# kakaobrain/rq-vae-transformer

Hardware: NVIDIA H100
Metric: 256x256 images/sec (ImageNet 1.4B RQ-Transformer, 8x8x4 codes, K=16384, top-k 1024, sample+decode) (higher is better)
Workload: dtype fp16

## Files before the change

include/rqb200.h:

```cpp
#ifndef RQB200_H
#define RQB200_H

#include <stddef.h>
#include <stdint.h>

#ifdef __cplusplus
extern "C" {
#endif

#define RQB200_OK 0
#define RQB200_EINVAL (-1)
#define RQB200_ECUDA (-2)
#define RQB200_ENODEV (-3)
#define RQB200_EWORKSPACE (-4)
#define RQB200_ESTATE (-5)

#define RQB200_F32 0
#define RQB200_BF16 1
#define RQB200_F16 2
#define RQB200_E4M3 3

#define RQB200_MODE_EXACT 0
#define RQB200_MODE_FAST 1

// ... 121 lines not shown
int64_t rqb200_vae_last_launches(const rqb200_vae* h);

int rqb200_dbg_gemm_tc(const void* W16, const void* X16, const float* bias, const float* residual, void* out,
                       int out_is_16, int gelu, float* partial, int N_out, int K, int B, int splits, int fmt, void* stream);
int rqb200_dbg_gemm_tc_fp8(const void* W8_packed, const float* scale, const void* X16, const float* bias, const float* residual,
                           void* out, int out_is_16, int gelu, float* partial, int N_out, int K, int B, int splits, void* stream);

int rqb200_dbg_rq_quantize(int form, const float* x, const float* codebook, int64_t N, int K, int C, int D, int64_t* codes,
                           float* quant_list, float* residual_out, void* stream);
int rqb200_dbg_rq_quantize_depthwise(int form, const float* x, const float* const* codebooks_host, const int32_t* K_host, int64_t N,
                                     int C, int D, int64_t* codes, float* quant_list, float* residual_out, void* stream);
int rqb200_dbg_sample_logits(int algo, const float* logits, const float* q, int B, int V, float temperature, int top_k,
                             float top_p, int64_t* out_idx, void* stream);

int rqb200_dbg_conv_tc(const void* X16, const void* W16, const void* X16lo, const void* W16lo, const float* bias,
                       const float* residual, float* out, int B, int H, int W, int Cin, int Cout, int ks, int out_nchw,
                       void* stream);

int rqb200_dbg_conv_tc_gn(const void* X16, const void* W16, const void* X16lo, const void* W16lo, const float* bias,
                          const float* residual, float* out, double* gn_part, int B, int H, int W, int Cin, int Cout, int ks,
                          int out_nchw, void* stream);

int rqb200_dbg_rows_gemm(const void* X16, const void* W16, const float* bias, const float* residual, float* out_f32, void* out_16,
                         int gelu, int fmt, int64_t M, int N_out, int K, void* stream);

int rqb200_dbg_log_prob_rows(const float* logits, int64_t ld, int V, int64_t rows, const int64_t* targets, float* out, void* stream);

int rqb200_dbg_attn_step(int form, const float* part, int S, const float* bqkv, void* kc, void* vc, void* att, int B, int E, int Tmax,
                         const int* t_dev, int t_host, int fmt, void* stream);
int rqb200_dbg_prefill_attn(const void* qkv, void* kc, void* vc, void* att, int G, int T, int E, int Tmax, int fmt, void* stream);
int rqb200_dbg_ln(int form, const float* x_in, const float* part, int S, const float* bias, const float* extra, float* x_out, const float* g,
                  const float* b, void* xn, int64_t rows, int E, int fmt, void* stream);
int rqb200_dbg_act_reduce(const float* part, int S, const float* bias, void* h, int B, int N, int fmt, void* stream);

int rqb200_dbg_vae_conv(const float* X, const void* Wt, int wdtype, const float* bias, const float* residual, float* out, int B, int H,
                        int W, int Cin, int Cout, int ks, int stride, int upsample, int in_nchw, int out_nchw, void* stream);
int rqb200_dbg_groupnorm(int form, const float* X, const float* gamma, const float* beta, float* Y, void* Y16, void* Y16lo,
                         double* stats_ws, int64_t ws_doubles, int B, int HW, int C, int silu, void* stream);
int rqb200_dbg_cast_f16(const float* X, void* Y16, void* Y16lo, int B, int H, int W, int C, int upsample, void* stream);
int rqb200_dbg_vae_attn(const float* qkv, float* out, int B, int HW, int C, void* stream);

#ifdef __cplusplus
}
#endif
#endif
```

rq-vae-transformer_b200/csrc/ar_fast.cu:

```cuda
#include <algorithm>
#include <cstring>
#include <string>
#include <vector>

#include "kernels.h"
#include "tc_common.cuh"

namespace rqb {

#define TR_IN(tr)  do { if ((tr) != nullptr && blockIdx.x == 0 && threadIdx.x == 0) (tr)[0] = tc::gtimer(); } while (0)
#define TR_DEP(tr) do { if ((tr) != nullptr && blockIdx.x == 0 && threadIdx.x == 0) (tr)[1] = tc::gtimer(); } while (0)
#define TR_OUT(tr) do { if ((tr) != nullptr && blockIdx.x == 0 && threadIdx.x == 0) { (tr)[2] = tc::gtimer(); (tr)[3] = (tr)[2]; } } while (0)

struct PrefetchList {
    const void* p[8];
    uint32_t bytes[8];
    int n;
};

template <int THREADS, int NCH>
__global__ void __launch_bounds__(THREADS)
ln_reduce_kernel(const float* __restrict__ x_in, const float* __restrict__ partial, int S, const float* __restrict__ bias,
                 const float* __restrict__ extra, float* __restrict__ x_out, const float* __restrict__ g,
                 const float* __restrict__ be, h16* __restrict__ xn, int B, int E, int bf, long long* tr, PrefetchList pf) {
    __shared__ float red[33];
    tc::pdl_launch_dependents();
    TR_IN(tr);
    if (blockIdx.x == 0 && threadIdx.x < pf.n) tc::bulk_prefetch_l2(pf.p[threadIdx.x], pf.bytes[threadIdx.x]);
    tc::pdl_wait();
    TR_DEP(tr);
    const int b = blockIdx.x;
    const int E4 = E >> 2;
    const int S12 = S < 12 ? S : 12;
    float4 v[NCH], gg[NCH], bb[NCH];
    float s = 0.f;
#pragma unroll
    for (int k = 0; k < NCH; k++) {
        const int e4 = threadIdx.x + k * THREADS;
        v[k] = make_float4(0.f, 0.f, 0.f, 0.f);
        if (e4 < E4) {
            float4 pr[12];
            if (xn) { gg[k] = reinterpret_cast<const float4*>(g)[e4]; bb[k] = reinterpret_cast<const float4*>(be)[e4]; }
#pragma unroll
            for (int i = 0; i < 12; i++)
                if (i < S12) pr[i] = reinterpret_cast<const float4*>(partial + ((int64_t)i * B + b) * E)[e4];
            if (x_in) v[k] = reinterpret_cast<const float4*>(x_in + (int64_t)b * E)[e4];
            if (bias) { float4 t = reinterpret_cast<const float4*>(bias)[e4]; v[k].x += t.x; v[k].y += t.y; v[k].z += t.z; v[k].w += t.w; }
#pragma unroll
            for (int i = 0; i < 12; i++)
                if (i < S12) { v[k].x += pr[i].x; v[k].y += pr[i].y; v[k].z += pr[i].z; v[k].w += pr[i].w; }
            for (int i = 12; i < S; i++) {
                float4 p0 = reinterpret_cast<const float4*>(partial + ((int64_t)i * B + b) * E)[e4];
                v[k].x += p0.x; v[k].y += p0.y; v[k].z += p0.z; v[k].w += p0.w;
            }
            if (extra) { float4 t = reinterpret_cast<const float4*>(extra)[e4]; v[k].x += t.x; v[k].y += t.y; v[k].z += t.z; v[k].w += t.w; }
            if (x_out) reinterpret_cast<float4*>(x_out + (int64_t)b * E)[e4] = v[k];
            s += (v[k].x + v[k].y) + (v[k].z + v[k].w);
        }
    }
    if (xn) {
        const float mean = block_sum(s, red) / (float)E;
        if (tr != nullptr && blockIdx.x == 0 && threadIdx.x == 0) tr[2] = tc::gtimer();
        float q = 0.f;
#pragma unroll
        for (int k = 0; k < NCH; k++)
            if (threadIdx.x + k * THREADS < E4) {
                const float d0 = v[k].x - mean, d1 = v[k].y - mean, d2 = v[k].z - mean, d3 = v[k].w - mean;
                q = fmaf(d0, d0, q); q = fmaf(d1, d1, q); q = fmaf(d2, d2, q); q = fmaf(d3, d3, q);
            }
        const float rstd = rsqrtf(block_sum(q, red) / (float)E + 1e-5f);
#pragma unroll
        for (int k = 0; k < NCH; k++) {
            const int e4 = threadIdx.x + k * THREADS;
            if (e4 < E4) {
                uint2 pk;
                pk.x = pack_h16x2((v[k].x - mean) * rstd * gg[k].x + bb[k].x, (v[k].y - mean) * rstd * gg[k].y + bb[k].y, bf);
                pk.y = pack_h16x2((v[k].z - mean) * rstd * gg[k].z + bb[k].z, (v[k].w - mean) * rstd * gg[k].w + bb[k].w, bf);
                reinterpret_cast<uint2*>(xn + (int64_t)b * E)[e4] = pk;
            }
        }
        if (tr != nullptr && blockIdx.x == 0 && threadIdx.x == 0) tr[3] = tc::gtimer();
    } else {
        TR_OUT(tr);
    }
}

template <int NV>
__global__ void __launch_bounds__(256)
ln_rows_kernel(const float* __restrict__ x_in, const float* __restrict__ extra, float* __restrict__ x_out, const float* __restrict__ g,
               const float* __restrict__ be, h16* __restrict__ xn, int64_t M, int E, int bf) {
    tc::pdl_launch_dependents();
    tc::pdl_wait();
    const int lane = threadIdx.x & 31;
// ... 157 lines not shown
    m = warp_max(m);
    if (tr != nullptr && blockIdx.x == 0 && threadIdx.x == 0) tr[2] = tc::gtimer();
    float sum = 0.f;
    for (int j = lane; j < t; j += 32) {
        float e = __expf(ps[j] - m);
        ps[j] = e;
        sum += e;
    }
    const float e_new = __expf(s_new - m);
    sum = warp_sum(sum) + e_new;
    __syncwarp();
    const float inv = 1.0f / sum;
    float2 o = make_float2(e_new * vf.x, e_new * vf.y);
    for (int j0 = 0; j0 < t; j0 += 64) {
        if (j0 > 0) {
#pragma unroll
            for (int u = 0; u < 64; u++)
                raw[u] = (j0 + u < t) ? *reinterpret_cast<const uint32_t*>(vb + (int64_t)(j0 + u) * 64 + 2 * lane) : 0u;
        }
#pragma unroll
        for (int u = 0; u < 64; u++)
            if (j0 + u < t) {
                const float2 vv = unpack_h16x2(raw[u], bf);
                o.x = fmaf(ps[j0 + u], vv.x, o.x);
                o.y = fmaf(ps[j0 + u], vv.y, o.y);
            }
    }
    *reinterpret_cast<uint32_t*>(att + (int64_t)b * E + c) = pack_h16x2(o.x * inv, o.y * inv, bf);
    }
    if (tr != nullptr && blockIdx.x == 0 && threadIdx.x == 0) tr[3] = tc::gtimer();
}

constexpr int AF2_MAXROWS = 320;
static size_t attn2_smem(int rows) { return (size_t)rows * 256 + ((size_t)rows + 64 * 3 + 4 * 64 + 8) * sizeof(float); }
__device__ __forceinline__ void cp_async16(uint32_t dst, const void* src) {
    asm volatile("cp.async.cg.shared.global [%0], [%1], 16;" ::"r"(dst), "l"(src) : "memory");
}
__global__ void __launch_bounds__(128, 11)
attn_fast2_kernel(const float* __restrict__ part, int S, const float* __restrict__ bqkv, h16* __restrict__ kc, h16* __restrict__ vc,
                  h16* __restrict__ att, int B, int E, int nh, int Tmax, int rows, const int* __restrict__ t_ptr, int t_host, int bf,
                  long long* tr) {
    extern __shared__ __align__(128) uint8_t af2_smem[];
    uint8_t* Ks = af2_smem;
    uint8_t* Vs = Ks + (size_t)rows * 128;
    float* ps = reinterpret_cast<float*>(Vs + (size_t)rows * 128);
    float* qs = ps + rows;
    float* kn = qs + 64;
    float* vn = kn + 64;
    float* ov = vn + 64;
    float* red = ov + 256;
    const int lane = threadIdx.x & 31, w = threadIdx.x >> 5;
    tc::pdl_launch_dependents();
    TR_IN(tr);
    tc::pdl_wait();
    TR_DEP(tr);
    const int b = blockIdx.x / nh, h = blockIdx.x % nh;
    const int t = t_ptr ? *t_ptr : t_host;
    h16* kb = kc + ((int64_t)(b * nh + h) * Tmax) * 64;
    h16* vb = vc + ((int64_t)(b * nh + h) * Tmax) * 64;
    {
        const uint32_t ks = tc::smem_u32(Ks), vs = tc::smem_u32(Vs);
        for (int i = threadIdx.x; i < t * 8; i += 128) {
            const int j = i >> 3, c = i & 7;
            const uint32_t off = (uint32_t)j * 128u + (uint32_t)((c ^ (j & 7)) << 4);
            cp_async16(ks + off, kb + (int64_t)j * 64 + c * 8);
            cp_async16(vs + off, vb + (int64_t)j * 64 + c * 8);
        }
        asm volatile("cp.async.commit_group;" ::: "memory");
    }
    if (w < 3) {
        const int c = h * 64 + 2 * lane;
        float2 a = make_float2(bqkv[w * E + c], bqkv[w * E + c + 1]);
#pragma unroll 4
        for (int s = 0; s < S; s++) {
            const float2 pp = *reinterpret_cast<const float2*>(part + ((int64_t)s * B + b) * 3 * E + w * E + c);
            a.x += pp.x; a.y += pp.y;
        }
        const uint32_t a2 = pack_h16x2(a.x, a.y, bf);
        const float2 af = unpack_h16x2(a2, bf);
        float* dst = w == 0 ? qs : (w == 1 ? kn : vn);
        dst[2 * lane] = af.x;
        dst[2 * lane + 1] = af.y;
        if (w == 1) *reinterpret_cast<uint32_t*>(kb + (int64_t)t * 64 + 2 * lane) = a2;
        if (w == 2) *reinterpret_cast<uint32_t*>(vb + (int64_t)t * 64 + 2 * lane) = a2;
    }
    asm volatile("cp.async.wait_group 0;" ::: "memory");
    __syncthreads();
    const float s_new = warp_sum(qs[2 * lane] * kn[2 * lane] + qs[2 * lane + 1] * kn[2 * lane + 1]) * 0.125f;
    float m = -INFINITY;
    {
        const int half = threadIdx.x & 1;
        for (int j0 = 0; j0 < t; j0 += 64) {
            const int j = j0 + (threadIdx.x >> 1);
            float acc = 0.f;
            if (j < t) {
#pragma unroll
                for (int i = 0; i < 4; i++) {
                    const int c = half * 4 + i;
                    const uint4 k4 = *reinterpret_cast<const uint4*>(Ks + (size_t)j * 128 + ((c ^ (j & 7)) << 4));
                    const float4 qa = *reinterpret_cast<const float4*>(qs + c * 8), qb = *reinterpret_cast<const float4*>(qs + c * 8 + 4);
                    float2 kk = unpack_h16x2(k4.x, bf);
                    acc = fmaf(qa.x, kk.x, acc); acc = fmaf(qa.y, kk.y, acc);
                    kk = unpack_h16x2(k4.y, bf);
                    acc = fmaf(qa.z, kk.x, acc); acc = fmaf(qa.w, kk.y, acc);
                    kk = unpack_h16x2(k4.z, bf);
                    acc = fmaf(qb.x, kk.x, acc); acc = fmaf(qb.y, kk.y, acc);
                    kk = unpack_h16x2(k4.w, bf);
                    acc = fmaf(qb.z, kk.x, acc); acc = fmaf(qb.w, kk.y, acc);
                }
            }
            acc += __shfl_xor_sync(0xffffffffu, acc, 1);
            acc *= 0.125f;
            if (j < t) {
                if (half == 0) ps[j] = acc;
                m = fmaxf(m, acc);
            }
        }
    }
    m = warp_max(m);
    if (lane == 0) red[w] = m;
    __syncthreads();
    m = fmaxf(fmaxf(fmaxf(red[0], red[1]), fmaxf(red[2], red[3])), s_new);
    if (tr != nullptr && blockIdx.x == 0 && threadIdx.x == 0) tr[2] = tc::gtimer();
    float sum = 0.f;
    for (int j = threadIdx.x; j < t; j += 128) {
        const float e = __expf(ps[j] - m);
        ps[j] = e;
        sum += e;
    }
    sum = warp_sum(sum);
    if (lane == 0) red[4 + w] = sum;
    __syncthreads();
    const float e_new = __expf(s_new - m);
    const float inv = 1.0f / ((((red[4] + red[5]) + red[6]) + red[7]) + e_new);
    float2 o = w == 0 ? make_float2(e_new * vn[2 * lane], e_new * vn[2 * lane + 1]) : make_float2(0.f, 0.f);
    for (int j = w; j < t; j += 4) {
        const uint32_t v2 = *reinterpret_cast<const uint32_t*>(Vs + (size_t)j * 128 + (((lane >> 2) ^ (j & 7)) << 4) + ((lane & 3) << 2));
        const float2 vv = unpack_h16x2(v2, bf);
        const float pj = ps[j];
        o.x = fmaf(pj, vv.x, o.x);
        o.y = fmaf(pj, vv.y, o.y);
    }
    ov[w * 64 + 2 * lane] = o.x;
    ov[w * 64 + 2 * lane + 1] = o.y;
    __syncthreads();
    if (w == 0) {
        const float ox = ((ov[2 * lane] + ov[64 + 2 * lane]) + ov[128 + 2 * lane]) + ov[192 + 2 * lane];
        const float oy = ((ov[2 * lane + 1] + ov[64 + 2 * lane + 1]) + ov[128 + 2 * lane + 1]) + ov[192 + 2 * lane + 1];
        *reinterpret_cast<uint32_t*>(att + (int64_t)b * E + h * 64 + 2 * lane) = pack_h16x2(ox * inv, oy * inv, bf);
    }
    if (tr != nullptr && blockIdx.x == 0 && threadIdx.x == 0) tr[3] = tc::gtimer();
}

template <bool BF>
__device__ __forceinline__ void pa_mma(float (&c)[4], const uint32_t (&a)[4], uint32_t b0, uint32_t b1) {
    if (BF)
        asm volatile("mma.sync.aligned.m16n8k16.row.col.f32.bf16.bf16.f32 {%0,%1,%2,%3}, {%4,%5,%6,%7}, {%8,%9}, {%0,%1,%2,%3};"
                     : "+f"(c[0]), "+f"(c[1]), "+f"(c[2]), "+f"(c[3]) : "r"(a[0]), "r"(a[1]), "r"(a[2]), "r"(a[3]), "r"(b0), "r"(b1));
    else
        asm volatile("mma.sync.aligned.m16n8k16.row.col.f32.f16.f16.f32 {%0,%1,%2,%3}, {%4,%5,%6,%7}, {%8,%9}, {%0,%1,%2,%3};"
                     : "+f"(c[0]), "+f"(c[1]), "+f"(c[2]), "+f"(c[3]) : "r"(a[0]), "r"(a[1]), "r"(a[2]), "r"(a[3]), "r"(b0), "r"(b1));
}
__device__ __forceinline__ void pa_ldsm4(uint32_t (&r)[4], uint32_t addr) {
    asm volatile("ldmatrix.sync.aligned.m8n8.x4.shared.b16 {%0,%1,%2,%3}, [%4];" : "=r"(r[0]), "=r"(r[1]), "=r"(r[2]), "=r"(r[3]) : "r"(addr));
}
__device__ __forceinline__ void pa_ldsm4_t(uint32_t (&r)[4], uint32_t addr) {
    asm volatile("ldmatrix.sync.aligned.m8n8.x4.trans.shared.b16 {%0,%1,%2,%3}, [%4];" : "=r"(r[0]), "=r"(r[1]), "=r"(r[2]), "=r"(r[3]) : "r"(addr));
}
// ... 354 lines not shown
    w.kc_body = a.take<h16>(per_body * c.n_body);
    w.vc_body = a.take<h16>(per_body * c.n_body);
    w.kc_head = a.take<h16>(per_head * c.n_head_layers);
    w.vc_head = a.take<h16>(per_head * c.n_head_layers);
    w.Mmax = f.batched_prefill ? (int64_t)B * prefill_tmax(c) : 0;
    const int64_t Mp = w.Mmax ? w.Mmax + 128 : 0;
    w.PX = a.take<float>(Mp * E);
    w.PXN = a.take<h16>(Mp * E);
    w.PQKV = a.take<h16>(Mp * 3 * E);
    w.PATT = a.take<h16>(Mp * E);
    w.PH = a.take<h16>(Mp * 4 * E);
    w.PS = a.take<h16>(w.Mmax * c.code_dim);
    if (ws) *ws = w;
    return a.off + 256;
}

static int gemm_w(const ArFast& f, const StreamedWeight& w, const CUtensorMap& tx, GemmTcParams p, bool pdl, cudaStream_t st) {
    p.fmt = f.bf; p.ld_out = w.N_out;
    return launch_gemm_tc(w, tx, p, pdl, st);
}

static int gemm(const ArFast& f, const char* name, const StreamedWeight& w, const CUtensorMap& tx, int B, int splits, int mode, const float* bias,
                float bias_scale, void* out, float* partial, const float* residual, int64_t ld_res, const int* res_row_ptr,
                int64_t res_row_stride, cudaStream_t st) {
    GemmTcParams p = {};
    p.B = B; p.splits = splits; p.mode = mode;
    p.bias = bias; p.bias_scale = bias_scale; p.out = out; p.partial = partial;
    p.residual = residual; p.ld_res = ld_res; p.res_row_ptr = res_row_ptr; p.res_row_stride = res_row_stride;
    p.trace = tr_slot(f, name);
    return gemm_w(f, w, tx, p, f.use_pdl, st);
}


static int ln(int rows, const float* x_in, const float* partial, int S, const float* bias, const float* extra, float* x_out, const float* g,
              const float* be, h16* xn, int E, int bf, bool pdl, long long* tr, const PrefetchList& pf, cudaStream_t st) {
    return launch_pdl(ln_reduce_kernel<384, 3>, dim3((unsigned)rows), dim3(384), (size_t)0, st, pdl, x_in, partial, S, bias, extra, x_out,
                      g, be, xn, rows, E, bf, tr, pf);
}

static int attn_form(int Tmax) { return Tmax >= 16 && Tmax - 1 <= AF2_MAXROWS ? 2 : 1; }

static int attn(int form, const float* part, int S, const float* bqkv, h16* kc, h16* vc, h16* att, int B, int E, int Tmax, const int* t_ptr,
                int t_host, int bf, bool pdl, long long* tr, cudaStream_t st) {
    const int nh = E / 64;
    if (form == 0) form = attn_form(Tmax);
    if (form == 2) {
        const int rows = (Tmax - 1 + 7) & ~7;
        RQB_ENSURE_SMEM(attn2_smem(AF2_MAXROWS), attn_fast2_kernel);
        {
            static std::atomic<uint64_t> carve{0};
            int dev = 0;
            RQB_CUDA(cudaGetDevice(&dev));
            if (!(carve.load(std::memory_order_acquire) & (1ull << (dev & 63)))) {
                RQB_CUDA(cudaFuncSetAttribute(attn_fast2_kernel, cudaFuncAttributePreferredSharedMemoryCarveout, 100));
                carve.fetch_or(1ull << (dev & 63), std::memory_order_release);
            }
        }
        return launch_pdl(attn_fast2_kernel, dim3((unsigned)(B * nh)), dim3(128), attn2_smem(rows), st, pdl, part, S, bqkv, kc, vc, att, B, E,
                          nh, Tmax, rows, t_ptr, t_host, bf, tr);
    }
    const size_t smem = (size_t)(4 * ((Tmax + 31) & ~31)) * sizeof(float);
    return launch_pdl(attn_fast_kernel, dim3((unsigned)ceil_div(B * nh, 4)), dim3(128), smem, st, pdl, part, S, bqkv, kc, vc, att, B, E, nh,
                      Tmax, t_ptr, t_host, bf, tr);
}

static int act_reduce(const float* partial, int S, const float* bias, h16* h, int B, int N, int bf, bool pdl, long long* tr, cudaStream_t st) {
    return launch_pdl(act_reduce_kernel, dim3((unsigned)std::min<int64_t>(ceil_div((int64_t)B * N / 4, 256), 1184)), dim3(256), (size_t)0, st,
                      pdl, partial, S, bias, h, B, N, bf, tr);
}

static int fast_stack(const ArFast& f, const std::vector<rqb200_block_weights>& blocks, const std::vector<FastLayer>& maps,
                      FastWs& ws, float* x, const float* pending_extra, const float* x_src, h16* kc, h16* vc, int Tmax,
                      const int* t_ptr, int t_host, const float* fin_g, const float* fin_b, cudaStream_t st) {
    const rqb200_ar_config& c = f.cfg;
    const int E = c.embed_dim, B = f.B;
    const int64_t per = (int64_t)B * c.n_head * Tmax * 64;
    const float* nof = nullptr;
    for (size_t l = 0; l < blocks.size(); l++) {
        const rqb200_block_weights& bw = blocks[l];
        const bool first = l == 0;
        const bool pend = l > 0;
        PrefetchList pf = {};
        if (l + 1 < blocks.size()) {
            const rqb200_block_weights& nx = blocks[l + 1];
            const void* ptrs[8] = {nx.ln1_w, nx.ln1_b, nx.bqkv, nx.bproj, nx.ln2_w, nx.ln2_b, nx.b1, bw.b2};
            const uint32_t words[8] = {(uint32_t)E, (uint32_t)E, (uint32_t)(3 * E), (uint32_t)E, (uint32_t)E, (uint32_t)E, (uint32_t)(4 * E),
                                       (uint32_t)E};
            for (int i = 0; i < 8; i++) { pf.p[i] = ptrs[i]; pf.bytes[i] = words[i] * 4u; }
            pf.n = 8;
        }
        RQB_TRY(ln(B, first ? x_src : x, pend ? ws.P : nof, pend ? f.split_fc2 : 0, pend ? blocks[l - 1].b2 : nof, first ? pending_extra : nof,
                   x, bw.ln1_w, bw.ln1_b, ws.XN, E, f.bf, f.use_pdl, tr_slot(f, "ln1"), pf, st));
        RQB_TRY(gemm(f, "qkv", maps[l].qkv, f.tx_xn, B, f.split_qkv, GT_PARTIAL, nullptr, 1.f, nullptr, ws.P, nullptr, 0, nullptr, 0, st));
        RQB_TRY(attn(0, ws.P, f.split_qkv, bw.bqkv, kc + per * l, vc + per * l, ws.ATT, B, E, Tmax, t_ptr, t_host, f.bf, f.use_pdl,
                     tr_slot(f, "attn"), st));
// ... 586 lines not shown
        return fail(RQB200_EINVAL, "dbg_prefill_attn: need fmt 0..1, G >= 1, 1 <= T <= 2048, E % 64 == 0");
    if (!qkv || !att || !kc != !vc) return fail(RQB200_EINVAL, "dbg_prefill_attn: null qkv / att, or only one of kc / vc");
    if (kc && T > Tmax) return fail(RQB200_EINVAL, "dbg_prefill_attn: T > Tmax");
    if (rqb200_device_count() <= 0) return fail(RQB200_ENODEV, "dbg_prefill_attn: no CUDA device");
    return prefill_attn((const h16*)qkv, (h16*)kc, (h16*)vc, (h16*)att, G, T, E, Tmax, fmt, false, (cudaStream_t)stream);
}

extern "C" int rqb200_dbg_ln(int form, const float* x_in, const float* partial, int S, const float* bias, const float* extra, float* x_out,
                             const float* g, const float* b, void* xn, int64_t rows, int E, int fmt, void* stream) {
    using namespace rqb;
    if (form < 0 || form > 2 || fmt < 0 || fmt > 1 || rows < 1 || rows > INT32_MAX || S < 0 || E < 128 || E % 128 || E > 4608)
        return fail(RQB200_EINVAL, "dbg_ln: need form 0..2, fmt 0..1, 1 <= rows < 2^31, S >= 0, E % 128 == 0, E <= 4608");
    if ((S > 0 && !partial) || (xn && (!g || !b))) return fail(RQB200_EINVAL, "dbg_ln: null partial, or xn without g / b");
    if (form != 1 && (S > 0 || partial || bias || !x_in))
        return fail(RQB200_EINVAL, "dbg_ln: forms 0 and 2 (the batched passes' LayerNorm) take x_in and no partials or bias");
    int dev = 0, n_sm = 0;
    if (rqb200_device_count() <= 0 || cudaGetDevice(&dev) != cudaSuccess ||
        cudaDeviceGetAttribute(&n_sm, cudaDevAttrMultiProcessorCount, dev) != cudaSuccess)
        return fail(RQB200_ENODEV, "dbg_ln: no CUDA device");
    const cudaStream_t st = (cudaStream_t)stream;
    if (form == 1) return ln((int)rows, x_in, partial, S, bias, extra, x_out, g, b, (h16*)xn, E, fmt, false, nullptr, PrefetchList{}, st);
    if (form == 2) return ln_rows_warp(rows, x_in, extra, x_out, g, b, (h16*)xn, E, fmt, n_sm, st);
    return ln_rows(rows, x_in, extra, x_out, g, b, (h16*)xn, E, fmt, n_sm, st);
}

extern "C" int rqb200_dbg_act_reduce(const float* partial, int S, const float* bias, void* h, int B, int N, int fmt, void* stream) {
    using namespace rqb;
    if (fmt < 0 || fmt > 1 || S < 0 || B < 1 || N < 4 || N % 4)
        return fail(RQB200_EINVAL, "dbg_act_reduce: need fmt 0..1, S >= 0, B >= 1, N % 4 == 0");
    if (!bias || !h || (S > 0 && !partial)) return fail(RQB200_EINVAL, "dbg_act_reduce: null argument");
    if (rqb200_device_count() <= 0) return fail(RQB200_ENODEV, "dbg_act_reduce: no CUDA device");
    return act_reduce(partial, S, bias, (h16*)h, B, N, fmt, false, nullptr, (cudaStream_t)stream);
}
```

rq-vae-transformer_b200/csrc/gemm_tc.cu:

```cuda
#include "kernels.h"
#include "tc_common.cuh"
#include <cudaTypedefs.h>
#include <cstdlib>

namespace rqb {

static int get_encode_fn(PFN_cuTensorMapEncodeTiled_v12000* fn) {
    static PFN_cuTensorMapEncodeTiled_v12000 cached = nullptr;
    if (!cached) {
        void* p = nullptr;
        cudaDriverEntryPointQueryResult q;
        cudaError_t e = cudaGetDriverEntryPoint("cuTensorMapEncodeTiled", &p, cudaEnableDefault, &q);
        if (e != cudaSuccess || q != cudaDriverEntryPointSuccess || !p)
            return fail(RQB200_ECUDA, "cuTensorMapEncodeTiled entry point not available");
        cached = (PFN_cuTensorMapEncodeTiled_v12000)p;
    }
    *fn = cached;
    return 0;
}

int make_tmap_2d(CUtensorMap* out, const void* base, int elem_bytes_log2, uint64_t inner, uint64_t outer,
                 uint64_t row_stride_bytes, uint32_t box_inner, uint32_t box_outer) {
    PFN_cuTensorMapEncodeTiled_v12000 enc;
    RQB_TRY(get_encode_fn(&enc));
// ... 254 lines not shown
        typename F::Frag none;
        for (int i = 0; i < nkb; i++) {
            const int s = i % STAGES;
            tc::mbar_wait(&full[s], (i / STAGES) & 1);
            tc::mbar_wait(&xfull[s], (i / STAGES) & 1);
            F::template kblock<BN>(acc, none, smem + s * STAGE_BYTES, wg, t, p.fmt, i == 0);
            tc::wgmma_commit();
            tc::wgmma_wait<1>();
            if (i > 0 && lane == 0) tc::mbar_arrive(&empty[(i - 1) % STAGES]);
        }
    }
    tc::wgmma_wait<0>();
    tc::acc_fence(acc);
    if (nkb > 0 && lane == 0) tc::mbar_arrive(&empty[(nkb - 1) % STAGES]);
    F::scale(acc, rs);

    tc::pdl_wait();
    if (tr && t == 0) p.trace[2] = tc::gtimer();
    const int nb = (p.B - m0) < BN ? (p.B - m0) : BN;
    const int n_base = tile * 128;
    tc::drain_acc<BN, CW, 0>(acc, stage, wg, t, [&p, n_base, split, m0, nb](const float (&v)[16], int r, int col0) {
        const int n = n_base + r;
        switch (p.mode) {
            case GT_PARTIAL: gt_epilogue<GT_PARTIAL>(p, v, n, split, m0, nb, col0); break;
            case GT_F32: gt_epilogue<GT_F32>(p, v, n, split, m0, nb, col0); break;
            case GT_H16: gt_epilogue<GT_H16>(p, v, n, split, m0, nb, col0); break;
            default: gt_epilogue<GT_H16_GELU>(p, v, n, split, m0, nb, col0); break;
        }
    });
    if (tr && t == 0) p.trace[3] = tc::gtimer();
}

template <int BN, int WF>
static int launch_gemm_tc_t(const typename GtFormat<WF>::Arg& w, const CUtensorMap& tmX, const GemmTcParams& p, bool pdl,
                            cudaStream_t st) {
    using F = GtFormat<WF>;
    constexpr size_t smem = (size_t)F::stages(BN) * (F::A_BYTES + BN * 128) + 128 * ((BN < 32 ? BN : 32) + 4) * 4 + 1024 + 512;
    static_assert(smem <= 227 * 1024, "gemm_tc: shared memory budget");
    RQB_ENSURE_SMEM(smem, gemm_tc_kernel<BN, WF>);
    return launch_pdl(gemm_tc_kernel<BN, WF>, dim3((unsigned)(ceil_div(p.N_out, 128) * p.splits), (unsigned)ceil_div(p.B, BN)),
                      dim3(GT_THREADS), smem, st, pdl, w, tmX, p);
}

template <int WF>
static int launch_gemm_tc_bn(const typename GtFormat<WF>::Arg& w, const CUtensorMap& tmX, const GemmTcParams& p, int bn, bool pdl,
                             cudaStream_t st) {
    switch (bn) {
        case 16: return launch_gemm_tc_t<16, WF>(w, tmX, p, pdl, st);
        case 32: return launch_gemm_tc_t<32, WF>(w, tmX, p, pdl, st);
        case 64: return launch_gemm_tc_t<64, WF>(w, tmX, p, pdl, st);
        case 128: return launch_gemm_tc_t<128, WF>(w, tmX, p, pdl, st);
        default: return launch_gemm_tc_t<(WF == GT_E4M3 ? 128 : 256), WF>(w, tmX, p, pdl, st);
    }
}

int make_streamed_weight(StreamedWeight* out, bool e4m3, const void* w, const float* scale, int N_out, int K) {
    *out = StreamedWeight{};
    out->N_out = N_out;
    out->K = K;
    if (e4m3) {
        if (w == nullptr || scale == nullptr || (reinterpret_cast<uintptr_t>(w) & 15) != 0)
            return fail(RQB200_EINVAL, "gemm_tc: packed E4M3 weights must be 16-byte aligned, scales non-null");
        out->q8 = static_cast<const uint8_t*>(w);
        out->s8 = scale;
        return 0;
    }
    out->w16 = w;
    return make_tmap_2d(&out->tm, w, 1, (uint64_t)K, (uint64_t)N_out, (uint64_t)K * 2, 64, 128);
}

int launch_gemm_tc(const StreamedWeight& w, const CUtensorMap& tmX, GemmTcParams p, bool pdl, cudaStream_t st) {
    p.N_out = w.N_out;
    p.K = w.K;
    if (p.K % 64 != 0 || p.N_out % 128 != 0) return fail(RQB200_EINVAL, "gemm_tc: need K % 64 == 0 and N_out % 128 == 0");
    if (p.B < 1) return fail(RQB200_EINVAL, "gemm_tc: no activation rows");
    if (p.splits < 1 || p.splits > p.K / 64) return fail(RQB200_EINVAL, "gemm_tc: bad split count");
    if (w.e4m3() && p.fmt != 0) return fail(RQB200_EINVAL, "gemm_tc: E4M3 weights take fp16 activations only");
    if (p.fmt != 0 && p.fmt != 1) return fail(RQB200_EINVAL, "gemm_tc: fmt must be 0 (fp16) or 1 (bf16)");
    if (p.B > 256 && p.mode == GT_PARTIAL) return fail(RQB200_EINVAL, "gemm_tc: split-K takes at most 256 activation rows");
    if (p.mode != GT_PARTIAL && p.splits != 1) return fail(RQB200_EINVAL, "gemm_tc: direct epilogues need splits == 1");
    const int bn = gemm_tc_chunk_rows(w, p.B);
    if (ceil_div(p.B, bn) > 65535) return fail(RQB200_EINVAL, "gemm_tc: more than 65535 row chunks");
    if (w.e4m3()) return launch_gemm_tc_bn<GT_E4M3>(GtE4m3Tiles{w.q8, w.s8}, tmX, p, bn, pdl, st);
    return launch_gemm_tc_bn<GT_W16>(w.tm, tmX, p, bn, pdl, st);
}
// ... 33 lines not shown
```

rq-vae-transformer_b200/csrc/kernels.h:

```cpp
#pragma once
#include <cuda.h>

#include "common.cuh"

namespace rqb {
constexpr int RQ_MAX_TABLES = 16;
struct RqTables {
    const float* cb[RQ_MAX_TABLES];
    int K[RQ_MAX_TABLES];
    int n;
    __host__ __device__ __forceinline__ int of(int depth) const { return n == 1 ? 0 : depth; }
};
int make_rq_tables(RqTables* out, const float* const* cb_host, const int32_t* K_host, int n);

int launch_rq_quantize(const float* x, const RqTables& tabs, int64_t N, int C, int D, int64_t* codes, float* quant_list,
                       float* resid_out, cudaStream_t st, int form = 0);
bool rq_quantize2_supported(int64_t N, const RqTables& tabs, int C);
int launch_rq_quantize2(const float* x, const RqTables& tabs, int64_t N, int C, int D, int64_t* codes, float* quant_list,
                        float* resid_out, cudaStream_t st);
int launch_rq_embed(const int64_t* codes, const RqTables& tabs, int64_t N, int D, int C, float* out, bool sum, cudaStream_t st);
int launch_sample(const float* logits, const float* q, int B, int V, float temperature, int top_k, float top_p,
                  int64_t* out_idx, const int64_t* force, int64_t out_stride, cudaStream_t st, int algo = 1, int cfg_n = 0,
                  float cfg_s = 0.f);
int launch_logprob_rows(const float* lg, int64_t ld, int V, int64_t rows, const int64_t* tgt, int64_t tgt_stride, float* out,
// ... 40 lines not shown
bool conv_tc_gn_fusable(int H, int W, int Cout, int ks, int stride);
int launch_rows_gemm_tc(const void* X16, const void* W16, const float* bias, const float* residual, float* out_f32, void* out_16,
                        int gelu, int fmt, int64_t M, int N_out, int K, cudaStream_t st);
int launch_groupnorm_f16(const float* X, const float* gamma, const float* beta, void* Y16, void* Y16lo, double* stats_ws, int B,
                         int HW, int C, int silu, cudaStream_t st, int fused_chunks = 0);
int launch_cast_f16(const float* X, void* Y16, void* Y16lo, int B, int H, int W, int C, int upsample, cudaStream_t st);
int make_tmap_4d_nhwc(CUtensorMap* out, const void* base, uint64_t C, uint64_t W, uint64_t H, uint64_t B, uint32_t box_c,
                      uint32_t box_w, uint32_t box_h, uint32_t box_b, uint32_t stride = 1);

enum GemmTcMode { GT_F32 = 0, GT_H16 = 1, GT_H16_GELU = 2, GT_PARTIAL = 3 };
struct GemmTcParams {
    int N_out, K, B, splits, mode;
    int fmt;
    const float* bias;
    float bias_scale;
    const float* residual;
    int64_t ld_res, res_row_stride;
    const int* res_row_ptr;
    int res_div;
    void* out;
    int64_t ld_out;
    float* partial;
    long long* trace;
};
struct StreamedWeight {
    int N_out = 0, K = 0;
    const void* w16 = nullptr;
    CUtensorMap tm;
    const uint8_t* q8 = nullptr;
    const float* s8 = nullptr;
    bool e4m3() const { return w16 == nullptr; }
};
int make_streamed_weight(StreamedWeight* out, bool e4m3, const void* w, const float* scale, int N_out, int K);
inline int gemm_tc_chunk_rows(const StreamedWeight& w, int64_t rows) {
    return rows <= 16 ? 16 : rows <= 32 ? 32 : rows <= 64 ? 64 : (rows <= 128 || w.e4m3()) ? 128 : 256;
}
int launch_gemm_tc(const StreamedWeight& w, const CUtensorMap& tmX, GemmTcParams p, bool pdl, cudaStream_t st);
int make_tmap_2d(CUtensorMap* out, const void* base, int elem_bytes_log2, uint64_t inner, uint64_t outer,
                 uint64_t row_stride_bytes, uint32_t box_inner, uint32_t box_outer);

struct StepState {
    int s;
    int idx;
    int step;
    int cfg_n;
    const int64_t* cond;
    int64_t* codes;
    const int64_t* force;
    const float* noise;
    float* logits_out;
    int64_t noise_stride;
    float temperature;
    float cfg_scale;
    int top_k[8];
    float top_p[8];
};
int launch_sample_dyn(const float* logits, const StepState* stt, int d, int B, int V, int HW, int D, cudaStream_t st, bool pdl);

struct ArFast;
ArFast* ar_fast_create(const rqb200_ar_config& cfg, const rqb200_ar_weights& w, const rqb200_block_weights* body,
                       const rqb200_block_weights* head);
void ar_fast_destroy(ArFast* f);
size_t ar_fast_workspace_bytes(const ArFast* f, int B);
int ar_fast_sample(ArFast* f, const int64_t* partial, const int64_t* cond, int B, int idx_begin, int idx_end, int resume,
                   float temperature, const int32_t* top_k, const float* top_p, const float* noise, int64_t noise_stride,
                   float* logits_out, const int64_t* force, int64_t* out, void* wsp, size_t ws_bytes, cudaStream_t st, int cfg_n = 0,
                   float cfg_s = 0.f);
int ar_fast_step(ArFast* f, const int64_t* xs, int64_t xs_stride, const int64_t* cond, int B, int idx, int d, int restart,
                 float* logits_out, void* wsp, size_t ws_bytes, cudaStream_t st);
size_t ar_fast_forward_workspace_bytes(const ArFast* f, int B);
// ... 8 lines not shown
```

rq-vae-transformer_b200/rqvae/_native.py:

```python
import ctypes as C
import os

import torch

_HERE = os.path.dirname(os.path.abspath(__file__))
LIB_PATH = os.environ.get("RQB200_LIB", os.path.join(os.path.dirname(_HERE), "csrc", "librqb200.so"))

OK, EINVAL, ECUDA, ENODEV, EWORKSPACE, ESTATE = 0, -1, -2, -3, -4, -5
F32, BF16, F16, E4M3 = 0, 1, 2, 3
MODE_EXACT, MODE_FAST = 0, 1
AR_NO_GRAPH, AR_NO_PDL, AR_TRACE, AR_SEQUENTIAL_PREFILL = 1, 2, 4, 32
EMB_TOK_INPUT, EMB_TOK_HEAD, EMB_NO_CUMSUM, EMB_TUPLE, EMB_CLS_PER_DEPTH = 1, 2, 4, 8, 16
_DT = {torch.float32: F32, torch.bfloat16: BF16, torch.float16: F16}

c_f32p, c_i64p, c_vp = C.c_void_p, C.c_void_p, C.c_void_p


class BlockWeights(C.Structure):
    _fields_ = [(n, C.c_void_p) for n in ("wqkv", "wproj", "w1", "w2", "bqkv", "bproj", "b1", "b2",
                                          "ln1_w", "ln1_b", "ln2_w", "ln2_b", "sqkv", "sproj", "s1", "s2")]


class ArConfig(C.Structure):
    _fields_ = [(n, C.c_int32) for n in ("embed_dim", "n_head", "n_body", "n_head_layers", "vocab", "H", "W", "D",
# ... 72 lines not shown
    L.rqb200_ar_forward_workspace_bytes.argtypes = [C.c_void_p, C.c_int]
    L.rqb200_ar_forward.argtypes = [C.c_void_p, C.c_void_p, C.c_void_p, C.c_int, C.c_void_p, C.c_void_p, C.c_void_p, C.c_size_t,
                                    C.c_void_p]
    L.rqb200_ar_log_prob_workspace_bytes.restype = C.c_size_t
    L.rqb200_ar_log_prob_workspace_bytes.argtypes = [C.c_void_p, C.c_int]
    L.rqb200_ar_log_prob.argtypes = L.rqb200_ar_forward.argtypes
    L.rqb200_dbg_log_prob_rows.argtypes = [C.c_void_p, C.c_int64, C.c_int, C.c_int64, C.c_void_p, C.c_void_p, C.c_void_p]
    L.rqb200_ar_trace.argtypes = [C.c_void_p, C.c_void_p, C.c_int, C.c_char_p, C.c_int]
    L.rqb200_ar_last_launches.restype = C.c_int64
    L.rqb200_ar_last_launches.argtypes = [C.c_void_p]
    L.rqb200_vae_create.restype = C.c_void_p
    L.rqb200_vae_create.argtypes = [C.POINTER(VaeConfig)]
    L.rqb200_vae_destroy.argtypes = [C.c_void_p]
    L.rqb200_vae_destroy.restype = None
    L.rqb200_vae_set_tensor.argtypes = [C.c_void_p, C.c_char_p, C.c_void_p, C.c_int, C.c_int64]
    L.rqb200_vae_finalize.argtypes = [C.c_void_p]
    L.rqb200_vae_workspace_bytes.restype = C.c_size_t
    L.rqb200_vae_workspace_bytes.argtypes = [C.c_void_p, C.c_int]
    for fn in (L.rqb200_vae_decode, L.rqb200_vae_decode_code, L.rqb200_vae_encode):
        fn.argtypes = [C.c_void_p, C.c_void_p, C.c_int, C.c_void_p, C.c_void_p, C.c_size_t, C.c_void_p]
    L.rqb200_vae_last_launches.restype = C.c_int64
    L.rqb200_vae_last_launches.argtypes = [C.c_void_p]
    L.rqb200_dbg_gemm_tc.argtypes = [C.c_void_p, C.c_void_p, C.c_void_p, C.c_void_p, C.c_void_p, C.c_int, C.c_int, C.c_void_p,
                                     C.c_int, C.c_int, C.c_int, C.c_int, C.c_int, C.c_void_p]
    L.rqb200_dbg_gemm_tc_fp8.argtypes = [C.c_void_p] * 6 + [C.c_int, C.c_int, C.c_void_p] + [C.c_int] * 4 + [C.c_void_p]
    L.rqb200_dbg_conv_tc.argtypes = [C.c_void_p, C.c_void_p, C.c_void_p, C.c_void_p, C.c_void_p, C.c_void_p, C.c_void_p, C.c_int,
                                     C.c_int, C.c_int, C.c_int, C.c_int, C.c_int, C.c_int, C.c_void_p]
    L.rqb200_dbg_conv_tc_gn.argtypes = [C.c_void_p] * 8 + [C.c_int] * 7 + [C.c_void_p]
    L.rqb200_dbg_attn_step.argtypes = [C.c_int, C.c_void_p, C.c_int] + [C.c_void_p] * 4 + [C.c_int] * 3 + [C.c_void_p] + [C.c_int] * 2 + \
                                      [C.c_void_p]
    L.rqb200_dbg_prefill_attn.argtypes = [C.c_void_p] * 4 + [C.c_int] * 5 + [C.c_void_p]
    L.rqb200_dbg_ln.argtypes = [C.c_int, C.c_void_p, C.c_void_p, C.c_int] + [C.c_void_p] * 6 + [C.c_int64, C.c_int, C.c_int, C.c_void_p]
    L.rqb200_dbg_act_reduce.argtypes = [C.c_void_p, C.c_int, C.c_void_p, C.c_void_p] + [C.c_int] * 3 + [C.c_void_p]
    L.rqb200_dbg_vae_conv.argtypes = [C.c_void_p, C.c_void_p, C.c_int] + [C.c_void_p] * 3 + [C.c_int] * 10 + [C.c_void_p]
    L.rqb200_dbg_groupnorm.argtypes = [C.c_int] + [C.c_void_p] * 7 + [C.c_int64] + [C.c_int] * 4 + [C.c_void_p]
    L.rqb200_dbg_cast_f16.argtypes = [C.c_void_p] * 3 + [C.c_int] * 5 + [C.c_void_p]
    L.rqb200_dbg_vae_attn.argtypes = [C.c_void_p] * 2 + [C.c_int] * 3 + [C.c_void_p]
    _lib = L
    return L


EXPORTS = ["rqb200_last_error", "rqb200_version", "rqb200_device_count", "rqb200_rq_quantize", "rqb200_rq_embed_sum",
           "rqb200_rq_embed_depth", "rqb200_rq_soft_codes", "rqb200_sample_logits", "rqb200_ar_create", "rqb200_ar_destroy",
           "rqb200_ar_workspace_bytes", "rqb200_ar_sample", "rqb200_ar_sample_span", "rqb200_ar_sample_span_cfg", "rqb200_ar_step", "rqb200_ar_forward",
           "rqb200_ar_forward_workspace_bytes", "rqb200_ar_trace", "rqb200_ar_last_launches", "rqb200_vae_create",
           "rqb200_vae_destroy", "rqb200_vae_set_tensor", "rqb200_vae_finalize", "rqb200_vae_workspace_bytes",
           "rqb200_vae_decode", "rqb200_vae_decode_code", "rqb200_vae_encode", "rqb200_vae_last_launches",
           "rqb200_dbg_gemm_tc", "rqb200_dbg_gemm_tc_fp8", "rqb200_dbg_conv_tc", "rqb200_dbg_conv_tc_gn", "rqb200_dbg_rq_quantize", "rqb200_dbg_sample_logits",
           "rqb200_dbg_rows_gemm", "rqb200_rq_quantize_depthwise", "rqb200_rq_embed_sum_depthwise",
           "rqb200_rq_embed_depth_depthwise", "rqb200_dbg_rq_quantize_depthwise", "rqb200_ar_log_prob",
           "rqb200_ar_log_prob_workspace_bytes", "rqb200_dbg_log_prob_rows", "rqb200_dbg_attn_step", "rqb200_dbg_prefill_attn",
           "rqb200_dbg_ln", "rqb200_dbg_act_reduce", "rqb200_dbg_vae_conv", "rqb200_dbg_groupnorm", "rqb200_dbg_cast_f16",
           "rqb200_dbg_vae_attn"]


def check(rc, what=""):
    if rc != 0:
        raise NativeError("rqb200 %s failed (%d): %s" % (what, rc, lib().rqb200_last_error().decode()))


def require_cuda(*tensors):
    for t in tensors:
        if t is not None and not t.is_cuda:
            raise NativeError("rqb200: tensor on %s -- this engine has no CPU path; move the model and inputs to a "
                              "CUDA device" % t.device)


def stream_ptr(device=None):
    return C.c_void_p(torch.cuda.current_stream(device).cuda_stream)


def ptr(t):
    return C.c_void_p(t.data_ptr()) if t is not None else C.c_void_p(0)


def dtype_code(t):
    return _DT[t.dtype]


def default_precision():
    return os.environ.get("RQB200_PRECISION", "auto")


def fast_dtype():
    return torch.bfloat16 if os.environ.get("RQB200_FAST_DTYPE", "fp16").lower() in ("bf16", "bfloat16") else torch.float16
# ... 72 lines not shown
```

Measured before the change: 189.3.

## Raise decode-step kernel residency and overlap attention cache loads with PDL wait

Specializes the layer-norm reduce kernel by embedding width (NCH 1/2/3) with a min-blocks launch bound, and defers gamma/beta loads until after the sum. This cuts register pressure so it can co-reside with the GEMM. The attention step kernel drops its reduction scratch to fit 12 blocks per SM and moves the PDL wait after the KV-cache cp.async prefetch, so cache loads overlap the previous kernel's tail. A debug residency query is added to check LN+GEMM co-residency. The risks are spills from the tighter launch bounds and a wrong early read if the cache rows being prefetched are written upstream.

Measured after the change: 194.9 (median of 6 runs). 1.03x the previous value.

```diff
diff --git a/include/rqb200.h b/include/rqb200.h
--- a/include/rqb200.h
+++ b/include/rqb200.h
@@ -177,6 +177,7 @@
 int rqb200_dbg_ln(int form, const float* x_in, const float* part, int S, const float* bias, const float* extra, float* x_out, const float* g,
                   const float* b, void* xn, int64_t rows, int E, int fmt, void* stream);
 int rqb200_dbg_act_reduce(const float* part, int S, const float* bias, void* h, int B, int N, int fmt, void* stream);
+int rqb200_dbg_step_residency(int B, int E, int Tmax, int e4m3, int* out);
 
 int rqb200_dbg_vae_conv(const float* X, const void* Wt, int wdtype, const float* bias, const float* residual, float* out, int B, int H,
                         int W, int Cin, int Cout, int ks, int stride, int upsample, int in_nchw, int out_nchw, void* stream);
diff --git a/rq-vae-transformer_b200/csrc/ar_fast.cu b/rq-vae-transformer_b200/csrc/ar_fast.cu
--- a/rq-vae-transformer_b200/csrc/ar_fast.cu
+++ b/rq-vae-transformer_b200/csrc/ar_fast.cu
@@ -19,10 +19,11 @@
 };
 
 template <int THREADS, int NCH>
-__global__ void __launch_bounds__(THREADS)
+__global__ void __launch_bounds__(THREADS, NCH <= 2 ? 2 : 1)
 ln_reduce_kernel(const float* __restrict__ x_in, const float* __restrict__ partial, int S, const float* __restrict__ bias,
                  const float* __restrict__ extra, float* __restrict__ x_out, const float* __restrict__ g,
-                 const float* __restrict__ be, h16* __restrict__ xn, int B, int E, int bf, long long* tr, PrefetchList pf) {
+                 const float* __restrict__ be, h16* __restrict__ xn, int B, int E, int bf, long long* tr,
+                 const __grid_constant__ PrefetchList pf) {
     __shared__ float red[33];
     tc::pdl_launch_dependents();
     TR_IN(tr);
@@ -40,7 +41,6 @@
         v[k] = make_float4(0.f, 0.f, 0.f, 0.f);
         if (e4 < E4) {
             float4 pr[12];
-            if (xn) { gg[k] = reinterpret_cast<const float4*>(g)[e4]; bb[k] = reinterpret_cast<const float4*>(be)[e4]; }
 #pragma unroll
             for (int i = 0; i < 12; i++)
                 if (i < S12) pr[i] = reinterpret_cast<const float4*>(partial + ((int64_t)i * B + b) * E)[e4];
@@ -59,6 +59,11 @@
         }
     }
     if (xn) {
+#pragma unroll
+        for (int k = 0; k < NCH; k++) {
+            const int e4 = threadIdx.x + k * THREADS;
+            if (e4 < E4) { gg[k] = reinterpret_cast<const float4*>(g)[e4]; bb[k] = reinterpret_cast<const float4*>(be)[e4]; }
+        }
         const float mean = block_sum(s, red) / (float)E;
         if (tr != nullptr && blockIdx.x == 0 && threadIdx.x == 0) tr[2] = tc::gtimer();
         float q = 0.f;
@@ -282,11 +287,11 @@
 }
 
 constexpr int AF2_MAXROWS = 320;
-static size_t attn2_smem(int rows) { return (size_t)rows * 256 + ((size_t)rows + 64 * 3 + 4 * 64 + 8) * sizeof(float); }
+static size_t attn2_smem(int rows) { return (size_t)rows * 256 + ((size_t)rows + 64 * 3 + 4 * 64) * sizeof(float); }
 __device__ __forceinline__ void cp_async16(uint32_t dst, const void* src) {
     asm volatile("cp.async.cg.shared.global [%0], [%1], 16;" ::"r"(dst), "l"(src) : "memory");
 }
-__global__ void __launch_bounds__(128, 11)
+__global__ void __launch_bounds__(128, 12)
 attn_fast2_kernel(const float* __restrict__ part, int S, const float* __restrict__ bqkv, h16* __restrict__ kc, h16* __restrict__ vc,
                   h16* __restrict__ att, int B, int E, int nh, int Tmax, int rows, const int* __restrict__ t_ptr, int t_host, int bf,
                   long long* tr) {
@@ -298,12 +303,10 @@
     float* kn = qs + 64;
     float* vn = kn + 64;
     float* ov = vn + 64;
-    float* red = ov + 256;
+    float* red = ov;
     const int lane = threadIdx.x & 31, w = threadIdx.x >> 5;
     tc::pdl_launch_dependents();
     TR_IN(tr);
-    tc::pdl_wait();
-    TR_DEP(tr);
     const int b = blockIdx.x / nh, h = blockIdx.x % nh;
     const int t = t_ptr ? *t_ptr : t_host;
     h16* kb = kc + ((int64_t)(b * nh + h) * Tmax) * 64;
@@ -318,6 +321,8 @@
         }
         asm volatile("cp.async.commit_group;" ::: "memory");
     }
+    tc::pdl_wait();
+    TR_DEP(tr);
     if (w < 3) {
         const int c = h * 64 + 2 * lane;
         float2 a = make_float2(bqkv[w * E + c], bqkv[w * E + c + 1]);
@@ -381,9 +386,13 @@
     sum = warp_sum(sum);
     if (lane == 0) red[4 + w] = sum;
     __syncthreads();
-    const float e_new = __expf(s_new - m);
-    const float inv = 1.0f / ((((red[4] + red[5]) + red[6]) + red[7]) + e_new);
-    float2 o = w == 0 ? make_float2(e_new * vn[2 * lane], e_new * vn[2 * lane + 1]) : make_float2(0.f, 0.f);
+    float2 o = make_float2(0.f, 0.f);
+    float inv = 0.f;
+    if (w == 0) {
+        const float e_new = __expf(s_new - m);
+        inv = 1.0f / ((((red[4] + red[5]) + red[6]) + red[7]) + e_new);
+        o = make_float2(e_new * vn[2 * lane], e_new * vn[2 * lane + 1]);
+    }
     for (int j = w; j < t; j += 4) {
         const uint32_t v2 = *reinterpret_cast<const uint32_t*>(Vs + (size_t)j * 128 + (((lane >> 2) ^ (j & 7)) << 4) + ((lane & 3) << 2));
         const float2 vv = unpack_h16x2(v2, bf);
@@ -804,35 +813,47 @@
 }
 
 
+constexpr int LN_THREADS = 384;
+using LnReduceFn = void (*)(const float*, const float*, int, const float*, const float*, float*, const float*, const float*, h16*, int, int,
+                            int, long long*, PrefetchList);
+static LnReduceFn ln_kernel(int E) {
+    return E <= LN_THREADS * 4 ? ln_reduce_kernel<LN_THREADS, 1> : E <= LN_THREADS * 8 ? ln_reduce_kernel<LN_THREADS, 2>
+                                                                                       : ln_reduce_kernel<LN_THREADS, 3>;
+}
 static int ln(int rows, const float* x_in, const float* partial, int S, const float* bias, const float* extra, float* x_out, const float* g,
               const float* be, h16* xn, int E, int bf, bool pdl, long long* tr, const PrefetchList& pf, cudaStream_t st) {
-    return launch_pdl(ln_reduce_kernel<384, 3>, dim3((unsigned)rows), dim3(384), (size_t)0, st, pdl, x_in, partial, S, bias, extra, x_out,
-                      g, be, xn, rows, E, bf, tr, pf);
+    return launch_pdl(ln_kernel(E), dim3((unsigned)rows), dim3(LN_THREADS), (size_t)0, st, pdl, x_in, partial, S, bias, extra, x_out, g, be,
+                      xn, rows, E, bf, tr, pf);
 }
 
 static int attn_form(int Tmax) { return Tmax >= 16 && Tmax - 1 <= AF2_MAXROWS ? 2 : 1; }
+
+static int attn2_rows(int Tmax) { return (Tmax - 1 + 7) & ~7; }
+static size_t attn1_smem(int Tmax) { return (size_t)(4 * ((Tmax + 31) & ~31)) * sizeof(float); }
+
+static int attn2_prepare() {
+    RQB_ENSURE_SMEM(attn2_smem(AF2_MAXROWS), attn_fast2_kernel);
+    static std::atomic<uint64_t> carve{0};
+    int dev = 0;
+    RQB_CUDA(cudaGetDevice(&dev));
+    if (!(carve.load(std::memory_order_acquire) & (1ull << (dev & 63)))) {
+        RQB_CUDA(cudaFuncSetAttribute(attn_fast2_kernel, cudaFuncAttributePreferredSharedMemoryCarveout, 100));
+        carve.fetch_or(1ull << (dev & 63), std::memory_order_release);
+    }
+    return 0;
+}
 
 static int attn(int form, const float* part, int S, const float* bqkv, h16* kc, h16* vc, h16* att, int B, int E, int Tmax, const int* t_ptr,
                 int t_host, int bf, bool pdl, long long* tr, cudaStream_t st) {
     const int nh = E / 64;
     if (form == 0) form = attn_form(Tmax);
     if (form == 2) {
-        const int rows = (Tmax - 1 + 7) & ~7;
-        RQB_ENSURE_SMEM(attn2_smem(AF2_MAXROWS), attn_fast2_kernel);
-        {
-            static std::atomic<uint64_t> carve{0};
-            int dev = 0;
-            RQB_CUDA(cudaGetDevice(&dev));
-            if (!(carve.load(std::memory_order_acquire) & (1ull << (dev & 63)))) {
-                RQB_CUDA(cudaFuncSetAttribute(attn_fast2_kernel, cudaFuncAttributePreferredSharedMemoryCarveout, 100));
-                carve.fetch_or(1ull << (dev & 63), std::memory_order_release);
-            }
-        }
+        const int rows = attn2_rows(Tmax);
+        RQB_TRY(attn2_prepare());
         return launch_pdl(attn_fast2_kernel, dim3((unsigned)(B * nh)), dim3(128), attn2_smem(rows), st, pdl, part, S, bqkv, kc, vc, att, B, E,
                           nh, Tmax, rows, t_ptr, t_host, bf, tr);
     }
-    const size_t smem = (size_t)(4 * ((Tmax + 31) & ~31)) * sizeof(float);
-    return launch_pdl(attn_fast_kernel, dim3((unsigned)ceil_div(B * nh, 4)), dim3(128), smem, st, pdl, part, S, bqkv, kc, vc, att, B, E, nh,
+    return launch_pdl(attn_fast_kernel, dim3((unsigned)ceil_div(B * nh, 4)), dim3(128), attn1_smem(Tmax), st, pdl, part, S, bqkv, kc, vc, att, B, E, nh,
                       Tmax, t_ptr, t_host, bf, tr);
 }
 
@@ -1485,3 +1506,36 @@
     if (rqb200_device_count() <= 0) return fail(RQB200_ENODEV, "dbg_act_reduce: no CUDA device");
     return act_reduce(partial, S, bias, (h16*)h, B, N, fmt, false, nullptr, (cudaStream_t)stream);
 }
+
+extern "C" int rqb200_dbg_step_residency(int B, int E, int Tmax, int e4m3, int* out) {
+    using namespace rqb;
+    if (B < 1 || B > 256 || E < 128 || E % 128 || E > 4608 || Tmax < 1 || Tmax > FAST_MAXT || e4m3 < 0 || e4m3 > 1 || !out)
+        return fail(RQB200_EINVAL, "dbg_step_residency: need 1 <= B <= 256, E % 128 == 0, E <= 4608, 1 <= Tmax <= 2048, e4m3 0..1, out");
+    int dev = 0;
+    cudaDeviceProp prop;
+    if (rqb200_device_count() <= 0 || cudaGetDevice(&dev) != cudaSuccess || cudaGetDeviceProperties(&prop, dev) != cudaSuccess)
+        return fail(RQB200_ENODEV, "dbg_step_residency: no CUDA device");
+    int attn_per_sm = 0;
+    if (attn_form(Tmax) == 2) {
+        RQB_TRY(attn2_prepare());
+        RQB_CUDA(cudaOccupancyMaxActiveBlocksPerMultiprocessor(&attn_per_sm, attn_fast2_kernel, 128, attn2_smem(attn2_rows(Tmax))));
+    } else {
+        RQB_CUDA(cudaOccupancyMaxActiveBlocksPerMultiprocessor(&attn_per_sm, attn_fast_kernel, 128, attn1_smem(Tmax)));
+    }
+    const int bn = gemm_tc_chunk_rows(e4m3 != 0, B);
+    cudaFuncAttributes la, ga;
+    size_t g_dyn = 0;
+    int g_threads = 0;
+    RQB_CUDA(cudaFuncGetAttributes(&la, ln_kernel(E)));
+    RQB_TRY(gemm_tc_footprint(e4m3 != 0, bn, &ga, &g_dyn, &g_threads));
+    auto regs = [](const cudaFuncAttributes& a, int threads) { return (a.numRegs + 7) / 8 * 8 * 32 * ((threads + 31) / 32); };
+    const int ln_regs = regs(la, LN_THREADS), g_regs = regs(ga, g_threads);
+    const size_t ln_smem = la.sharedSizeBytes + prop.reservedSharedMemPerBlock;
+    const size_t g_smem = ga.sharedSizeBytes + g_dyn + prop.reservedSharedMemPerBlock;
+    const bool fits = ln_regs + g_regs <= prop.regsPerMultiprocessor && ln_smem + g_smem <= prop.sharedMemPerMultiprocessor &&
+                      LN_THREADS + g_threads <= prop.maxThreadsPerMultiProcessor;
+    const int vals[10] = {attn_per_sm, prop.multiProcessorCount, fits ? 1 : 0, ln_regs, g_regs, prop.regsPerMultiprocessor, (int)ln_smem,
+                          (int)g_smem, (int)prop.sharedMemPerMultiprocessor, bn};
+    memcpy(out, vals, sizeof(vals));
+    return 0;
+}
diff --git a/rq-vae-transformer_b200/csrc/gemm_tc.cu b/rq-vae-transformer_b200/csrc/gemm_tc.cu
--- a/rq-vae-transformer_b200/csrc/gemm_tc.cu
+++ b/rq-vae-transformer_b200/csrc/gemm_tc.cu
@@ -310,10 +310,14 @@
 }
 
 template <int BN, int WF>
+constexpr size_t gt_smem() {
+    return (size_t)GtFormat<WF>::stages(BN) * (GtFormat<WF>::A_BYTES + BN * 128) + 128 * ((BN < 32 ? BN : 32) + 4) * 4 + 1024 + 512;
+}
+
+template <int BN, int WF>
 static int launch_gemm_tc_t(const typename GtFormat<WF>::Arg& w, const CUtensorMap& tmX, const GemmTcParams& p, bool pdl,
                             cudaStream_t st) {
-    using F = GtFormat<WF>;
-    constexpr size_t smem = (size_t)F::stages(BN) * (F::A_BYTES + BN * 128) + 128 * ((BN < 32 ? BN : 32) + 4) * 4 + 1024 + 512;
+    constexpr size_t smem = gt_smem<BN, WF>();
     static_assert(smem <= 227 * 1024, "gemm_tc: shared memory budget");
     RQB_ENSURE_SMEM(smem, gemm_tc_kernel<BN, WF>);
     return launch_pdl(gemm_tc_kernel<BN, WF>, dim3((unsigned)(ceil_div(p.N_out, 128) * p.splits), (unsigned)ceil_div(p.B, BN)),
@@ -329,6 +333,29 @@
         case 64: return launch_gemm_tc_t<64, WF>(w, tmX, p, pdl, st);
         case 128: return launch_gemm_tc_t<128, WF>(w, tmX, p, pdl, st);
         default: return launch_gemm_tc_t<(WF == GT_E4M3 ? 128 : 256), WF>(w, tmX, p, pdl, st);
+    }
+}
+
+template <int BN, int WF>
+static int gemm_tc_footprint_t(cudaFuncAttributes* attr, size_t* smem, int* threads) {
+    *smem = gt_smem<BN, WF>();
+    *threads = GT_THREADS;
+    RQB_CUDA(cudaFuncGetAttributes(attr, gemm_tc_kernel<BN, WF>));
+    return 0;
+}
+
+int gemm_tc_footprint(bool e4m3, int bn, cudaFuncAttributes* attr, size_t* smem, int* threads) {
+    switch (bn * 2 + (e4m3 ? 1 : 0)) {
+        case 32: return gemm_tc_footprint_t<16, GT_W16>(attr, smem, threads);
+        case 33: return gemm_tc_footprint_t<16, GT_E4M3>(attr, smem, threads);
+        case 64: return gemm_tc_footprint_t<32, GT_W16>(attr, smem, threads);
+        case 65: return gemm_tc_footprint_t<32, GT_E4M3>(attr, smem, threads);
+        case 128: return gemm_tc_footprint_t<64, GT_W16>(attr, smem, threads);
+        case 129: return gemm_tc_footprint_t<64, GT_E4M3>(attr, smem, threads);
+        case 256: return gemm_tc_footprint_t<128, GT_W16>(attr, smem, threads);
+        case 257: return gemm_tc_footprint_t<128, GT_E4M3>(attr, smem, threads);
+        case 512: return gemm_tc_footprint_t<256, GT_W16>(attr, smem, threads);
+        default: return fail(RQB200_EINVAL, "gemm_tc_footprint: bn must be 16, 32, 64, 128 or (16-bit weights) 256");
     }
 }
 
diff --git a/rq-vae-transformer_b200/csrc/kernels.h b/rq-vae-transformer_b200/csrc/kernels.h
--- a/rq-vae-transformer_b200/csrc/kernels.h
+++ b/rq-vae-transformer_b200/csrc/kernels.h
@@ -96,10 +96,12 @@
     bool e4m3() const { return w16 == nullptr; }
 };
 int make_streamed_weight(StreamedWeight* out, bool e4m3, const void* w, const float* scale, int N_out, int K);
-inline int gemm_tc_chunk_rows(const StreamedWeight& w, int64_t rows) {
-    return rows <= 16 ? 16 : rows <= 32 ? 32 : rows <= 64 ? 64 : (rows <= 128 || w.e4m3()) ? 128 : 256;
+inline int gemm_tc_chunk_rows(bool e4m3, int64_t rows) {
+    return rows <= 16 ? 16 : rows <= 32 ? 32 : rows <= 64 ? 64 : (rows <= 128 || e4m3) ? 128 : 256;
 }
+inline int gemm_tc_chunk_rows(const StreamedWeight& w, int64_t rows) { return gemm_tc_chunk_rows(w.e4m3(), rows); }
 int launch_gemm_tc(const StreamedWeight& w, const CUtensorMap& tmX, GemmTcParams p, bool pdl, cudaStream_t st);
+int gemm_tc_footprint(bool e4m3, int bn, cudaFuncAttributes* attr, size_t* smem, int* threads);
 int make_tmap_2d(CUtensorMap* out, const void* base, int elem_bytes_log2, uint64_t inner, uint64_t outer,
                  uint64_t row_stride_bytes, uint32_t box_inner, uint32_t box_outer);
 
diff --git a/rq-vae-transformer_b200/rqvae/_native.py b/rq-vae-transformer_b200/rqvae/_native.py
--- a/rq-vae-transformer_b200/rqvae/_native.py
+++ b/rq-vae-transformer_b200/rqvae/_native.py
@@ -128,6 +128,7 @@
     L.rqb200_dbg_prefill_attn.argtypes = [C.c_void_p] * 4 + [C.c_int] * 5 + [C.c_void_p]
     L.rqb200_dbg_ln.argtypes = [C.c_int, C.c_void_p, C.c_void_p, C.c_int] + [C.c_void_p] * 6 + [C.c_int64, C.c_int, C.c_int, C.c_void_p]
     L.rqb200_dbg_act_reduce.argtypes = [C.c_void_p, C.c_int, C.c_void_p, C.c_void_p] + [C.c_int] * 3 + [C.c_void_p]
+    L.rqb200_dbg_step_residency.argtypes = [C.c_int] * 4 + [C.POINTER(C.c_int)]
     L.rqb200_dbg_vae_conv.argtypes = [C.c_void_p, C.c_void_p, C.c_int] + [C.c_void_p] * 3 + [C.c_int] * 10 + [C.c_void_p]
     L.rqb200_dbg_groupnorm.argtypes = [C.c_int] + [C.c_void_p] * 7 + [C.c_int64] + [C.c_int] * 4 + [C.c_void_p]
     L.rqb200_dbg_cast_f16.argtypes = [C.c_void_p] * 3 + [C.c_int] * 5 + [C.c_void_p]
@@ -146,7 +147,7 @@
            "rqb200_dbg_rows_gemm", "rqb200_rq_quantize_depthwise", "rqb200_rq_embed_sum_depthwise",
            "rqb200_rq_embed_depth_depthwise", "rqb200_dbg_rq_quantize_depthwise", "rqb200_ar_log_prob",
            "rqb200_ar_log_prob_workspace_bytes", "rqb200_dbg_log_prob_rows", "rqb200_dbg_attn_step", "rqb200_dbg_prefill_attn",
-           "rqb200_dbg_ln", "rqb200_dbg_act_reduce", "rqb200_dbg_vae_conv", "rqb200_dbg_groupnorm", "rqb200_dbg_cast_f16",
+           "rqb200_dbg_ln", "rqb200_dbg_act_reduce", "rqb200_dbg_step_residency", "rqb200_dbg_vae_conv", "rqb200_dbg_groupnorm", "rqb200_dbg_cast_f16",
            "rqb200_dbg_vae_attn"]
 
 
```
